# Drexubery/ViewCrafter

Hardware: NVIDIA H100
Metric: DDIM denoise-steps/sec @ 576x1024x25f (higher is better)
Workload: dtype f16 (fp32 accumulate; fp32 norms/softmax/update)

## Files before the change

viewcrafter_b200/csrc/attention.cu:

```cuda
#include <cstdlib>

#include "common.cuh"
#include "kernels.h"
#include "wgmma.cuh"

namespace vc {

struct AttnParams {
  CUtensorMap tmap_q, tmap_k, tmap_v;
  __half* out;
  int ldo;
  int Nq, Nk;
  int kv_shared;
  float scale_log2;
  int accumulate;
};

static constexpr int ATT_BM = 128, ATT_D = 64;
static constexpr int ATT_THREADS = 288;
static constexpr int ATT_Q_BYTES = ATT_BM * ATT_D * 2;

template <int BNK>
struct AttnCfg {
  static constexpr int KV_BYTES = BNK * ATT_D * 2;
  static constexpr int SMEM = ATT_Q_BYTES + 4 * KV_BYTES + 1024 + 256;
  static constexpr int MIN_CTAS = BNK == 64 ? 2 : 1;
};

__device__ __forceinline__ float ex2f(float x) {
  float y;
  asm("ex2.approx.ftz.f32 %0, %1;" : "=f"(y) : "f"(x));
  return y;
}

template <int BNK>
__global__ void __launch_bounds__(ATT_THREADS, AttnCfg<BNK>::MIN_CTAS) flash_attn_d64_kernel(const __grid_constant__ AttnParams p) {
  using Cfg = AttnCfg<BNK>;
  extern __shared__ uint8_t smem_raw[];
  uint8_t* smem = reinterpret_cast<uint8_t*>((reinterpret_cast<uintptr_t>(smem_raw) + 1023) & ~uintptr_t(1023));
  uint8_t* sQ = smem;
  uint8_t* sKV = smem + ATT_Q_BYTES;
  uint64_t* bars = reinterpret_cast<uint64_t*>(smem + ATT_Q_BYTES + 4 * Cfg::KV_BYTES);
  uint64_t* q_full = bars + 0;
  uint64_t* kv_full = bars + 1;
  uint64_t* kv_empty = bars + 3;

  const int warp = threadIdx.x >> 5, lane = threadIdx.x & 31;
  const int q0 = blockIdx.x * ATT_BM, head = blockIdx.y, b = blockIdx.z;
  const int bk = p.kv_shared ? 0 : b;
  const int ntiles = (p.Nk + BNK - 1) / BNK;

  if (threadIdx.x == 0) {
    tma_prefetch_desc(&p.tmap_q);
    tma_prefetch_desc(&p.tmap_k);
    tma_prefetch_desc(&p.tmap_v);
    mbar_init(q_full, 1);
    mbar_init(&kv_full[0], 1); mbar_init(&kv_full[1], 1);
    mbar_init(&kv_empty[0], 8); mbar_init(&kv_empty[1], 8);
    fence_barrier_init();
  }
  __syncthreads();

  if (warp == 8) {
    if (elect_one()) {
      mbar_expect_tx(q_full, ATT_Q_BYTES);
      tma_load_4d(sQ, &p.tmap_q, q_full, 0, head, q0, b);
    }
    __syncwarp();
    for (int j = 0; j < ntiles; ++j) {
      const int s = j & 1;
      uint8_t* sk = sKV + s * 2 * Cfg::KV_BYTES;
      if (j >= 2) mbar_wait(&kv_empty[s], ((j >> 1) - 1) & 1);
      if (elect_one()) {
        mbar_expect_tx(&kv_full[s], 2 * Cfg::KV_BYTES);
        tma_load_4d(sk, &p.tmap_k, &kv_full[s], 0, head, j * BNK, bk);
        tma_load_4d(sk + Cfg::KV_BYTES, &p.tmap_v, &kv_full[s], 0, head, j * BNK, bk);
      }
      __syncwarp();
    }
    return;
  }

  const int cw = warp >> 2, wl = warp & 3;
  const uint32_t aQ = smem_u32(sQ) + cw * (64 * ATT_D * 2);
  const float sl2 = p.scale_log2;
  float o[32];
#pragma unroll
  for (int i = 0; i < 32; ++i) o[i] = 0.f;
  float m[2] = {-INFINITY, -INFINITY}, l[2] = {0.f, 0.f};
  mbar_wait(q_full, 0);
  for (int j = 0; j < ntiles; ++j) {
    const int s = j & 1;
    const uint32_t aK = smem_u32(sKV + s * 2 * Cfg::KV_BYTES);
    const uint32_t aV = aK + Cfg::KV_BYTES;
    mbar_wait(&kv_full[s], (j >> 1) & 1);
    float sc[BNK / 2];
    wgmma_fence();
#pragma unroll
    for (int k = 0; k < ATT_D / 16; ++k) Wgmma<BNK>::ss(sc, wgmma_desc_sw128(aQ + 32 * k), wgmma_desc_sw128(aK + 32 * k), k > 0 ? 1 : 0);
    wgmma_commit();
    wgmma_wait<0>();
    wgmma_fence_regs(sc);

    const int valid = p.Nk - j * BNK;
    if (valid < BNK) {
#pragma unroll
      for (int i = 0; i < BNK / 2; ++i) {
        const int col = 8 * (i >> 2) + 2 * (lane & 3) + (i & 1);
        if (col >= valid) sc[i] = -INFINITY;
      }
    }
    float mx[2] = {-INFINITY, -INFINITY};
#pragma unroll
    for (int i = 0; i < BNK / 2; ++i) mx[(i >> 1) & 1] = fmaxf(mx[(i >> 1) & 1], sc[i]);
    float alpha[2], negm[2];
#pragma unroll
    for (int h = 0; h < 2; ++h) {
      mx[h] = fmaxf(mx[h], __shfl_xor_sync(0xffffffffu, mx[h], 1));
      mx[h] = fmaxf(mx[h], __shfl_xor_sync(0xffffffffu, mx[h], 2));
      const float mn = fmaxf(m[h], mx[h] * sl2);
      alpha[h] = ex2f(m[h] - mn);
      m[h] = mn;
      negm[h] = -mn;
      l[h] *= alpha[h];
    }
#pragma unroll
    for (int i = 0; i < 32; ++i) o[i] *= alpha[(i >> 1) & 1];
    uint32_t pa[BNK / 16][4];
#pragma unroll
    for (int kk = 0; kk < BNK / 16; ++kk) {
#pragma unroll
      for (int r = 0; r < 4; ++r) {
        const int i = (2 * kk + (r >> 1)) * 4 + 2 * (r & 1);
        const int h = r & 1;
        const float e0 = ex2f(fmaf(sc[i], sl2, negm[h])), e1 = ex2f(fmaf(sc[i + 1], sl2, negm[h]));
        l[h] += e0 + e1;
        pa[kk][r] = pack_half2(e0, e1);
      }
    }
    wgmma_fence();
#pragma unroll
    for (int kk = 0; kk < BNK / 16; ++kk) Wgmma<64, 1>::rs(o, pa[kk], wgmma_desc_sw128(aV + kk * 16 * 128), 1);
    wgmma_commit();
    wgmma_wait<0>();
    wgmma_fence_regs(o);
    __syncwarp();
    if (lane == 0) mbar_arrive(&kv_empty[s]);
  }

  float inv[2];
#pragma unroll
  for (int h = 0; h < 2; ++h) {
    float t = l[h];
    t += __shfl_xor_sync(0xffffffffu, t, 1);
    t += __shfl_xor_sync(0xffffffffu, t, 2);
    inv[h] = 1.f / t;
  }
#pragma unroll
  for (int h = 0; h < 2; ++h) {
    const int row = q0 + cw * 64 + 16 * wl + (lane >> 2) + 8 * h;
    if (row >= p.Nq) continue;
    __half* op = p.out + ((long long)b * p.Nq + row) * p.ldo + head * ATT_D + 2 * (lane & 3);
#pragma unroll
    for (int jj = 0; jj < 8; ++jj) {
      float v0 = o[jj * 4 + 2 * h] * inv[h], v1 = o[jj * 4 + 2 * h + 1] * inv[h];
      __half2* dst = reinterpret_cast<__half2*>(op + 8 * jj);
      if (p.accumulate) {
        const float2 t = __half22float2(*dst);
        v0 += t.x; v1 += t.y;
      }
      *dst = __floats2half2_rn(v0, v1);
    }
  }
}

static int bn64_mode() {
  static int mode = -2;
  if (mode == -2) { const char* e = getenv("VC_ATTN_BN64"); mode = !e ? -1 : (e[0] == '1' ? 1 : 0); }
  return mode;
}

template <int BNK>
static int launch_attn(const vc_attn_desc& d, cudaStream_t stream) {
  using Cfg = AttnCfg<BNK>;
  AttnParams p;
  memset(&p, 0, sizeof(p));
  {
    uint64_t dims[4] = {64, (uint64_t)d.heads, (uint64_t)d.Nq, (uint64_t)d.B};
    uint64_t str[3] = {128, (uint64_t)d.ldq * 2, (uint64_t)d.ldq * 2 * d.Nq};
    uint32_t box[4] = {64, 1, ATT_BM, 1};
    int rc = encode_tmap_f16(&p.tmap_q, d.q, 4, dims, str, box);
    if (rc) return rc;
  }
  const int shared = d.kv_batch_stride == 0;
  {
    uint64_t dims[4] = {64, (uint64_t)d.heads, (uint64_t)d.Nk, (uint64_t)(shared ? 1 : d.B)};
    uint64_t strk[3] = {128, (uint64_t)d.ldk * 2, (uint64_t)(shared ? (long long)d.ldk * d.Nk : d.kv_batch_stride) * 2};
    uint64_t strv[3] = {128, (uint64_t)d.ldv * 2, (uint64_t)(shared ? (long long)d.ldv * d.Nk : d.kv_batch_stride) * 2};
    uint32_t box[4] = {64, 1, (uint32_t)BNK, 1};
    int rc = encode_tmap_f16(&p.tmap_k, d.k, 4, dims, strk, box);
    if (rc) return rc;
    rc = encode_tmap_f16(&p.tmap_v, d.v, 4, dims, strv, box);
    if (rc) return rc;
  }
  p.out = static_cast<__half*>(d.out); p.ldo = d.ldo; p.Nq = d.Nq; p.Nk = d.Nk; p.kv_shared = shared;
  p.scale_log2 = d.scale * 1.4426950408889634f;
  p.accumulate = d.accumulate;
  static DeviceOnce configured;
  if (device_once_needed(configured)) {
    VC_CHECK_CUDA(cudaFuncSetAttribute(flash_attn_d64_kernel<BNK>, cudaFuncAttributeMaxDynamicSharedMemorySize, Cfg::SMEM));
    device_once_mark(configured);
  }
  dim3 grid((d.Nq + ATT_BM - 1) / ATT_BM, d.heads, d.B);
  flash_attn_d64_kernel<BNK><<<grid, ATT_THREADS, Cfg::SMEM, stream>>>(p);
  VC_CHECK_CUDA(cudaGetLastError());
  return VC_OK;
}

int flash_attn_d64(const vc_attn_desc& d, cudaStream_t stream) {
  VC_REQUIRE(d.q && d.k && d.v && d.out, "flash_attn: null pointer");
  VC_REQUIRE(d.Nq > 0 && d.Nk > 0 && d.B > 0 && d.heads > 0, "flash_attn: empty problem");
  VC_REQUIRE(d.ldq % 8 == 0 && d.ldk % 8 == 0 && d.ldv % 8 == 0 && d.ldo % 8 == 0, "flash_attn: pitches must be multiples of 8");
  VC_REQUIRE(d.kv_batch_stride % 8 == 0, "flash_attn: kv batch stride must be a multiple of 8");
  const int mode = bn64_mode();
  if (mode == 1 || (mode < 0 && d.Nk <= 1024)) return launch_attn<64>(d, stream);
  return launch_attn<128>(d, stream);
}

}
```

Before: 2.593.

## Add warp-specialized pipelined flash-attention kernel for the 128-wide KV tile path

Adds a new BNK=128 attention kernel. It uses producer warps with reduced registers (setmaxnreg), separate K and V full/empty barriers across 4 stages, and MMA warpgroups that overlap the next tile's QK^T wgmma with the current PV wgmma and softmax. It also skips the output rescale when alpha is 1 across the warp. The aim is to hide softmax latency and TMA waits behind tensor-core work, at the cost of more shared memory, 384 threads and higher register pressure. The BNK=64 path keeps the original kernel, with the softmax and store pulled out into shared helpers.

```diff
diff --git a/viewcrafter_b200/csrc/attention.cu b/viewcrafter_b200/csrc/attention.cu
--- a/viewcrafter_b200/csrc/attention.cu
+++ b/viewcrafter_b200/csrc/attention.cu
@@ -17,15 +17,18 @@
 };
 
 static constexpr int ATT_BM = 128, ATT_D = 64;
-static constexpr int ATT_THREADS = 288;
 static constexpr int ATT_Q_BYTES = ATT_BM * ATT_D * 2;
 
 template <int BNK>
 struct AttnCfg {
   static constexpr int KV_BYTES = BNK * ATT_D * 2;
-  static constexpr int SMEM = ATT_Q_BYTES + 4 * KV_BYTES + 1024 + 256;
+  static constexpr int STAGES = BNK == 64 ? 2 : 4;
+  static constexpr int THREADS = BNK == 64 ? 288 : 384;
+  static constexpr int SMEM = ATT_Q_BYTES + 2 * STAGES * KV_BYTES + 1024 + 256;
   static constexpr int MIN_CTAS = BNK == 64 ? 2 : 1;
 };
+static constexpr int ATT_LAUNCH_REGS = 168, ATT_PRODUCER_REGS = 24, ATT_MMA_REGS = 240;
+static_assert(128 * ATT_PRODUCER_REGS + 256 * ATT_MMA_REGS <= ATT_LAUNCH_REGS * AttnCfg<128>::THREADS, "register split exceeds the CTA's allocation");
 
 __device__ __forceinline__ float ex2f(float x) {
   float y;
@@ -34,13 +37,78 @@
 }
 
 template <int BNK>
-__global__ void __launch_bounds__(ATT_THREADS, AttnCfg<BNK>::MIN_CTAS) flash_attn_d64_kernel(const __grid_constant__ AttnParams p) {
+__device__ __forceinline__ void attn_softmax(float (&sc)[BNK / 2], int valid, float sl2, int lane, float (&m)[2], float (&l)[2],
+                                             float (&alpha)[2], uint32_t (&pa)[BNK / 16][4]) {
+  if (valid < BNK) {
+#pragma unroll
+    for (int i = 0; i < BNK / 2; ++i) {
+      const int col = 8 * (i >> 2) + 2 * (lane & 3) + (i & 1);
+      if (col >= valid) sc[i] = -INFINITY;
+    }
+  }
+  float mx[2] = {-INFINITY, -INFINITY};
+#pragma unroll
+  for (int i = 0; i < BNK / 2; ++i) mx[(i >> 1) & 1] = fmaxf(mx[(i >> 1) & 1], sc[i]);
+  float negm[2];
+#pragma unroll
+  for (int h = 0; h < 2; ++h) {
+    mx[h] = fmaxf(mx[h], __shfl_xor_sync(0xffffffffu, mx[h], 1));
+    mx[h] = fmaxf(mx[h], __shfl_xor_sync(0xffffffffu, mx[h], 2));
+    const float mn = fmaxf(m[h], mx[h] * sl2);
+    alpha[h] = ex2f(m[h] - mn);
+    m[h] = mn;
+    negm[h] = -mn;
+    l[h] *= alpha[h];
+  }
+#pragma unroll
+  for (int kk = 0; kk < BNK / 16; ++kk) {
+#pragma unroll
+    for (int r = 0; r < 4; ++r) {
+      const int i = (2 * kk + (r >> 1)) * 4 + 2 * (r & 1);
+      const int h = r & 1;
+      const float e0 = ex2f(fmaf(sc[i], sl2, negm[h])), e1 = ex2f(fmaf(sc[i + 1], sl2, negm[h]));
+      l[h] += e0 + e1;
+      pa[kk][r] = pack_half2(e0, e1);
+    }
+  }
+}
+
+__device__ __forceinline__ void attn_store(const AttnParams& p, const float (&o)[32], const float (&l)[2], int q0, int cw, int wl,
+                                           int lane, int head, int b) {
+  float inv[2];
+#pragma unroll
+  for (int h = 0; h < 2; ++h) {
+    float t = l[h];
+    t += __shfl_xor_sync(0xffffffffu, t, 1);
+    t += __shfl_xor_sync(0xffffffffu, t, 2);
+    inv[h] = 1.f / t;
+  }
+#pragma unroll
+  for (int h = 0; h < 2; ++h) {
+    const int row = q0 + cw * 64 + 16 * wl + (lane >> 2) + 8 * h;
+    if (row >= p.Nq) continue;
+    __half* op = p.out + ((long long)b * p.Nq + row) * p.ldo + head * ATT_D + 2 * (lane & 3);
+#pragma unroll
+    for (int jj = 0; jj < 8; ++jj) {
+      float v0 = o[jj * 4 + 2 * h] * inv[h], v1 = o[jj * 4 + 2 * h + 1] * inv[h];
+      __half2* dst = reinterpret_cast<__half2*>(op + 8 * jj);
+      if (p.accumulate) {
+        const float2 t = __half22float2(*dst);
+        v0 += t.x; v1 += t.y;
+      }
+      *dst = __floats2half2_rn(v0, v1);
+    }
+  }
+}
+
+template <int BNK>
+__global__ void __launch_bounds__(AttnCfg<BNK>::THREADS, AttnCfg<BNK>::MIN_CTAS) flash_attn_d64_kernel(const __grid_constant__ AttnParams p) {
   using Cfg = AttnCfg<BNK>;
   extern __shared__ uint8_t smem_raw[];
   uint8_t* smem = reinterpret_cast<uint8_t*>((reinterpret_cast<uintptr_t>(smem_raw) + 1023) & ~uintptr_t(1023));
   uint8_t* sQ = smem;
   uint8_t* sKV = smem + ATT_Q_BYTES;
-  uint64_t* bars = reinterpret_cast<uint64_t*>(smem + ATT_Q_BYTES + 4 * Cfg::KV_BYTES);
+  uint64_t* bars = reinterpret_cast<uint64_t*>(smem + ATT_Q_BYTES + 2 * Cfg::STAGES * Cfg::KV_BYTES);
   uint64_t* q_full = bars + 0;
   uint64_t* kv_full = bars + 1;
   uint64_t* kv_empty = bars + 3;
@@ -102,42 +170,11 @@
     wgmma_wait<0>();
     wgmma_fence_regs(sc);
 
-    const int valid = p.Nk - j * BNK;
-    if (valid < BNK) {
-#pragma unroll
-      for (int i = 0; i < BNK / 2; ++i) {
-        const int col = 8 * (i >> 2) + 2 * (lane & 3) + (i & 1);
-        if (col >= valid) sc[i] = -INFINITY;
-      }
-    }
-    float mx[2] = {-INFINITY, -INFINITY};
-#pragma unroll
-    for (int i = 0; i < BNK / 2; ++i) mx[(i >> 1) & 1] = fmaxf(mx[(i >> 1) & 1], sc[i]);
-    float alpha[2], negm[2];
-#pragma unroll
-    for (int h = 0; h < 2; ++h) {
-      mx[h] = fmaxf(mx[h], __shfl_xor_sync(0xffffffffu, mx[h], 1));
-      mx[h] = fmaxf(mx[h], __shfl_xor_sync(0xffffffffu, mx[h], 2));
-      const float mn = fmaxf(m[h], mx[h] * sl2);
-      alpha[h] = ex2f(m[h] - mn);
-      m[h] = mn;
-      negm[h] = -mn;
-      l[h] *= alpha[h];
-    }
+    float alpha[2];
+    uint32_t pa[BNK / 16][4];
+    attn_softmax<BNK>(sc, p.Nk - j * BNK, sl2, lane, m, l, alpha, pa);
 #pragma unroll
     for (int i = 0; i < 32; ++i) o[i] *= alpha[(i >> 1) & 1];
-    uint32_t pa[BNK / 16][4];
-#pragma unroll
-    for (int kk = 0; kk < BNK / 16; ++kk) {
-#pragma unroll
-      for (int r = 0; r < 4; ++r) {
-        const int i = (2 * kk + (r >> 1)) * 4 + 2 * (r & 1);
-        const int h = r & 1;
-        const float e0 = ex2f(fmaf(sc[i], sl2, negm[h])), e1 = ex2f(fmaf(sc[i + 1], sl2, negm[h]));
-        l[h] += e0 + e1;
-        pa[kk][r] = pack_half2(e0, e1);
-      }
-    }
     wgmma_fence();
 #pragma unroll
     for (int kk = 0; kk < BNK / 16; ++kk) Wgmma<64, 1>::rs(o, pa[kk], wgmma_desc_sw128(aV + kk * 16 * 128), 1);
@@ -147,31 +184,158 @@
     __syncwarp();
     if (lane == 0) mbar_arrive(&kv_empty[s]);
   }
-
-  float inv[2];
-#pragma unroll
-  for (int h = 0; h < 2; ++h) {
-    float t = l[h];
-    t += __shfl_xor_sync(0xffffffffu, t, 1);
-    t += __shfl_xor_sync(0xffffffffu, t, 2);
-    inv[h] = 1.f / t;
-  }
-#pragma unroll
-  for (int h = 0; h < 2; ++h) {
-    const int row = q0 + cw * 64 + 16 * wl + (lane >> 2) + 8 * h;
-    if (row >= p.Nq) continue;
-    __half* op = p.out + ((long long)b * p.Nq + row) * p.ldo + head * ATT_D + 2 * (lane & 3);
-#pragma unroll
-    for (int jj = 0; jj < 8; ++jj) {
-      float v0 = o[jj * 4 + 2 * h] * inv[h], v1 = o[jj * 4 + 2 * h + 1] * inv[h];
-      __half2* dst = reinterpret_cast<__half2*>(op + 8 * jj);
-      if (p.accumulate) {
-        const float2 t = __half22float2(*dst);
-        v0 += t.x; v1 += t.y;
+  attn_store(p, o, l, q0, cw, wl, lane, head, b);
+}
+
+__global__ void __launch_bounds__(AttnCfg<128>::THREADS, 1) flash_attn_d64_pipe_kernel(const __grid_constant__ AttnParams p) {
+  using Cfg = AttnCfg<128>;
+  constexpr int STAGES = Cfg::STAGES;
+  extern __shared__ uint8_t smem_raw[];
+  uint8_t* smem = reinterpret_cast<uint8_t*>((reinterpret_cast<uintptr_t>(smem_raw) + 1023) & ~uintptr_t(1023));
+  uint8_t* sQ = smem;
+  uint8_t* sK = smem + ATT_Q_BYTES;
+  uint8_t* sV = sK + STAGES * Cfg::KV_BYTES;
+  uint64_t* bars = reinterpret_cast<uint64_t*>(sV + STAGES * Cfg::KV_BYTES);
+  uint64_t* q_full = bars;
+  uint64_t* k_full = bars + 1;
+  uint64_t* v_full = k_full + STAGES;
+  uint64_t* k_empty = v_full + STAGES;
+  uint64_t* v_empty = k_empty + STAGES;
+
+  const int warp = threadIdx.x >> 5, lane = threadIdx.x & 31;
+  const int q0 = blockIdx.x * ATT_BM, head = blockIdx.y, b = blockIdx.z;
+  const int bk = p.kv_shared ? 0 : b;
+  const int ntiles = (p.Nk + 127) / 128;
+
+  if (threadIdx.x == 0) {
+    tma_prefetch_desc(&p.tmap_q);
+    tma_prefetch_desc(&p.tmap_k);
+    tma_prefetch_desc(&p.tmap_v);
+    mbar_init(q_full, 1);
+    for (int s = 0; s < STAGES; ++s) {
+      mbar_init(&k_full[s], 1);
+      mbar_init(&v_full[s], 1);
+      mbar_init(&k_empty[s], 8);
+      mbar_init(&v_empty[s], 8);
+    }
+    fence_barrier_init();
+  }
+  __syncthreads();
+
+  if (warp < 4) {
+    setmaxnreg_dec<ATT_PRODUCER_REGS>();
+    if (warp != 0) return;
+    if (elect_one()) {
+      mbar_expect_tx(q_full, ATT_Q_BYTES);
+      tma_load_4d(sQ, &p.tmap_q, q_full, 0, head, q0, b);
+    }
+    __syncwarp();
+    int s = 0;
+    uint32_t ph = 0;
+    for (int j = 0; j < ntiles; ++j) {
+      mbar_wait(&k_empty[s], ph ^ 1);
+      if (elect_one()) {
+        mbar_expect_tx(&k_full[s], Cfg::KV_BYTES);
+        tma_load_4d(sK + s * Cfg::KV_BYTES, &p.tmap_k, &k_full[s], 0, head, j * 128, bk);
       }
-      *dst = __floats2half2_rn(v0, v1);
-    }
-  }
+      __syncwarp();
+      mbar_wait(&v_empty[s], ph ^ 1);
+      if (elect_one()) {
+        mbar_expect_tx(&v_full[s], Cfg::KV_BYTES);
+        tma_load_4d(sV + s * Cfg::KV_BYTES, &p.tmap_v, &v_full[s], 0, head, j * 128, bk);
+      }
+      __syncwarp();
+      if (++s == STAGES) { s = 0; ph ^= 1; }
+    }
+    return;
+  }
+
+  setmaxnreg_inc<ATT_MMA_REGS>();
+  const int cw = (warp >> 2) - 1, wl = warp & 3;
+  const uint32_t aQ = smem_u32(sQ) + cw * (64 * ATT_D * 2);
+  const uint32_t aK0 = smem_u32(sK), aV0 = smem_u32(sV);
+  const float sl2 = p.scale_log2;
+  float o[32];
+#pragma unroll
+  for (int i = 0; i < 32; ++i) o[i] = 0.f;
+  float m[2] = {-INFINITY, -INFINITY}, l[2] = {0.f, 0.f}, alpha[2];
+  float sc[64];
+  uint32_t pa[8][4], pb[8][4];
+  int ks = 0, vs = 0;
+  uint32_t kph = 0, vph = 0;
+
+  const auto rescale = [&] {
+    if (!__all_sync(0xffffffffu, alpha[0] == 1.f && alpha[1] == 1.f)) {
+#pragma unroll
+      for (int i = 0; i < 32; ++i) o[i] *= alpha[(i >> 1) & 1];
+    }
+  };
+  const uint64_t dQ0 = wgmma_desc_sw128(aQ);
+  const auto issue_s = [&] {
+    uint64_t dQ = dQ0;
+    asm volatile("" : "+l"(dQ));
+    const uint64_t dK = wgmma_desc_sw128(aK0 + ks * Cfg::KV_BYTES);
+#pragma unroll
+    for (int k = 0; k < ATT_D / 16; ++k) Wgmma<128>::ss(sc, dQ + 2 * k, dK + 2 * k, k > 0 ? 1 : 0);
+    wgmma_commit();
+  };
+  const auto issue_pv = [&](uint32_t (&pc)[8][4]) {
+    const uint32_t aV = aV0 + vs * Cfg::KV_BYTES;
+#pragma unroll
+    for (int kk = 0; kk < 8; ++kk) Wgmma<64, 1>::rs(o, pc[kk], wgmma_desc_sw128(aV + kk * 16 * 128), 1);
+    wgmma_commit();
+  };
+  const auto release = [&](uint64_t* empty, int& slot, uint32_t& ph) {
+    __syncwarp();
+    if (lane == 0) mbar_arrive(&empty[slot]);
+    if (++slot == STAGES) { slot = 0; ph ^= 1; }
+  };
+  const auto keep_p = [&](uint32_t (&pc)[8][4]) {
+#pragma unroll
+    for (int kk = 0; kk < 8; ++kk)
+#pragma unroll
+      for (int r = 0; r < 4; ++r) asm volatile("" : "+r"(pc[kk][r])::"memory");
+  };
+  const auto step = [&](uint32_t (&pc)[8][4], uint32_t (&pn)[8][4], int j) {
+    mbar_wait(&k_full[ks], kph);
+    mbar_wait(&v_full[vs], vph);
+    wgmma_fence();
+    issue_s();
+    issue_pv(pc);
+    wgmma_wait<1>();
+    wgmma_fence_regs(sc);
+    release(k_empty, ks, kph);
+    attn_softmax<128>(sc, p.Nk - (j + 1) * 128, sl2, lane, m, l, alpha, pn);
+    wgmma_wait<0>();
+    wgmma_fence_regs(o);
+    keep_p(pc);
+    release(v_empty, vs, vph);
+    rescale();
+  };
+
+  mbar_wait(q_full, 0);
+  mbar_wait(&k_full[ks], kph);
+  wgmma_fence();
+  issue_s();
+  wgmma_wait<0>();
+  wgmma_fence_regs(sc);
+  release(k_empty, ks, kph);
+  attn_softmax<128>(sc, p.Nk, sl2, lane, m, l, alpha, pa);
+  int j = 0;
+  for (; j + 2 < ntiles; j += 2) {
+    step(pa, pb, j);
+    step(pb, pa, j + 1);
+  }
+  const bool in_b = j + 1 < ntiles;
+  if (in_b) step(pa, pb, j);
+  mbar_wait(&v_full[vs], vph);
+  wgmma_fence();
+  if (in_b) issue_pv(pb); else issue_pv(pa);
+  wgmma_wait<0>();
+  wgmma_fence_regs(o);
+  keep_p(pa);
+  keep_p(pb);
+  attn_store(p, o, l, q0, cw, wl, lane, head, b);
 }
 
 static int bn64_mode() {
@@ -206,13 +370,14 @@
   p.out = static_cast<__half*>(d.out); p.ldo = d.ldo; p.Nq = d.Nq; p.Nk = d.Nk; p.kv_shared = shared;
   p.scale_log2 = d.scale * 1.4426950408889634f;
   p.accumulate = d.accumulate;
+  void (*kernel)(const AttnParams) = BNK == 64 ? flash_attn_d64_kernel<64> : flash_attn_d64_pipe_kernel;
   static DeviceOnce configured;
   if (device_once_needed(configured)) {
-    VC_CHECK_CUDA(cudaFuncSetAttribute(flash_attn_d64_kernel<BNK>, cudaFuncAttributeMaxDynamicSharedMemorySize, Cfg::SMEM));
+    VC_CHECK_CUDA(cudaFuncSetAttribute(kernel, cudaFuncAttributeMaxDynamicSharedMemorySize, Cfg::SMEM));
     device_once_mark(configured);
   }
   dim3 grid((d.Nq + ATT_BM - 1) / ATT_BM, d.heads, d.B);
-  flash_attn_d64_kernel<BNK><<<grid, ATT_THREADS, Cfg::SMEM, stream>>>(p);
+  kernel<<<grid, Cfg::THREADS, Cfg::SMEM, stream>>>(p);
   VC_CHECK_CUDA(cudaGetLastError());
   return VC_OK;
 }
```

Result: faster. 2.636, median of 6 (+1.6%).
